# evanwang1990/FMwR

Hardware: AMD Instinct MI355X
Metric: training examples/sec, 10Mx1M sparse FM SGD (higher is better)
Workload: dtype f32

## Files before the change

fmwr_amd/_lib.py:

```python
import ctypes as C
import os

_PKG = os.path.dirname(os.path.abspath(__file__))
LIB_PATH = os.environ.get("FMX_LIB_PATH") or os.path.join(_PKG, "libfmx.so")

OK, ERR_INVALID, ERR_HIP, ERR_NOGPU, ERR_STATE = 0, 1, 2, 3, 4
TASK_CLASSIFICATION, TASK_REGRESSION, TASK_RANKING = 10, 20, 30
SOLVER_MCMC, SOLVER_ALS, SOLVER_SGD, SOLVER_FTRL, SOLVER_TDAP = 100, 200, 300, 500, 600
MODE_SEQUENTIAL, MODE_MINIBATCH = 0, 1
LINK_NONE, LINK_LOGISTIC, LINK_CLAMP, LINK_PROBIT = 0, 1, 2, 3
DIV_REL_SCORE, DIV_REL_MINMAX = 0, 1
SIM_COSINE, SIM_DOT = 0, 1
REDUCE_MEAN, REDUCE_SUM = 0, 1
COLUMNS_UNIFORM, COLUMNS_ZIPF = 1, 2
EVAL_LL, EVAL_AUC, EVAL_ACC, EVAL_RMSE, EVAL_MSE, EVAL_MAE = 0, 111, 222, 333, 444, 555
EVAL_PAIR_ACC, EVAL_BPR = 666, 777
KERNEL_ROWS_FORWARD, KERNEL_COLS_UPDATE, KERNEL_SCALAR, KERNEL_SEQ, KERNEL_ALS_SWEEP = 0, 1, 2, 3, 4

SYMBOLS = [
    "fmx_last_error", "fmx_device_count", "fmx_config_default", "fmx_engine_create", "fmx_engine_destroy", "fmx_set_params",
    "fmx_get_params", "fmx_engine_save", "fmx_engine_load", "fmx_matrix_from_rlist", "fmx_matrix_from_dgc", "fmx_matrix_from_csr", "fmx_matrix_synthetic", "fmx_matrix_synthetic_fields", "fmx_matrix_synthetic_iid", "fmx_matrix_synthetic_ragged", "fmx_matrix_synthetic_values", "fmx_train_stream", "fmx_matrix_set_labels", "fmx_matrix_set_fields", "fmx_matrix_destroy",
    "fmx_matrix_info", "fmx_matrix_export", "fmx_matrix_scales", "fmx_matrix_normalize", "fmx_predict", "fmx_train", "fmx_train_grid", "fmx_train_order", "fmx_num_batches",
    "fmx_step", "fmx_grad", "fmx_grad_buffer", "fmx_grad_elem_bytes", "fmx_grad_layout", "fmx_grad_begin", "fmx_grad_chunk", "fmx_apply_chunk", "fmx_apply", "fmx_sync", "fmx_stream", "fmx_predict_device",
    "fmx_als_plan_info", "fmx_als_tiled_info", "fmx_als_order_info", "fmx_als_carry_q", "fmx_als_vsweep", "fmx_mcmc_vsweep", "fmx_als_train", "fmx_mcmc_train", "fmx_mcmc_train_from", "fmx_mcmc_v_hyper", "fmx_evaluate", "fmx_train_tracked", "fmx_trace_size", "fmx_trace_get", "fmx_trace_params",
# ... 19 lines not shown
]
COLUMNS_BY_ROWS, COLUMNS_BY_ENTRIES = 0, 1
RARE_DROP, RARE_BUCKET = 0, 1
COMBINE_KEEP, COMBINE_SUM, COMBINE_FIRST = 0, 1, 2
COLUMN_DROP = 0xFFFFFFFF
SPLIT_ROWS, SPLIT_WITHIN_GROUPS, SPLIT_GROUPS = 0, 1, 2
SPLIT_ORDER_HASH, SPLIT_ORDER_TAIL = 0, 1
SPLIT_NO_PART = 0xFFFFFFFF
MET_VALUES, MET_COUNTS = 6, 4
MET_AUC, MET_LOGLOSS, MET_ACCURACY, MET_BRIER, MET_MEAN_PRED, MET_MEAN_LABEL = 0, 1, 2, 3, 4, 5
MET_MSE, MET_RMSE, MET_MAE, MET_MEAN_ERR = 0, 1, 2, 3
MET_ROWS, MET_POSITIVES, MET_PAIRS2, MET_CORRECT = 0, 1, 2, 3
CAL_NONE, CAL_PLATT, CAL_STEPS = 0, 1, 2
BINS_WIDTH, BINS_MASS = 0, 1
CAL_VALUES = 4
CAL_ECE, CAL_MCE, CAL_BRIER, CAL_LOGLOSS = 0, 1, 2, 3


TEST_HOOKS = ["fmx_debug_fail_next_plan_build", "fmx_debug_fail_next_comm_init", "fmx_debug_lose_next_seq_multiplier", "fmx_debug_stall_next_persistent_sweep",
              "fmx_debug_contrib_summary_chunk", "fmx_debug_foldin_slab", "fmx_debug_heldout_limits", "fmx_debug_pairs_hard_chunk", "fmx_debug_lists_limits", "fmx_debug_diversify_limits", "fmx_debug_neighbors_limits", "fmx_debug_interactions_limits", "fmx_debug_metrics_limits", "fmx_debug_take_limits", "fmx_debug_calibrate_limits", "fmx_debug_columns_limits", "fmx_debug_matrix_flags", "fmx_debug_cols_launches",
              "fmx_debug_long_launches", "fmx_debug_rows_launches", "fmx_debug_rows_merged_launches",
              "fmx_debug_rows_sched_launches", "fmx_debug_rows_sched_id_limit", "fmx_debug_rows_sched_export",
              "fmx_debug_rows_pace_launches", "fmx_debug_rows_pace_trace",
              "fmx_debug_rows_clock_launches", "fmx_debug_rows_clock_records_of", "fmx_debug_rows_clock_poison"]


class Config(C.Structure):
    _fields_ = [
        ("struct_size", C.c_uint32), ("task", C.c_int32), ("solver", C.c_int32), ("num_factor", C.c_int32),
        ("keep_w0", C.c_int32), ("keep_w1", C.c_int32),
        ("l2_w0", C.c_double), ("l1_w1", C.c_double), ("l2_w1", C.c_double), ("l1_v", C.c_double), ("l2_v", C.c_double),
        ("learn_rate", C.c_double),
        ("alpha_w", C.c_double), ("alpha_v", C.c_double), ("beta_w", C.c_double), ("beta_v", C.c_double),
        ("random_step", C.c_int32), ("mode", C.c_int32), ("batch_rows", C.c_int64),
        ("min_target", C.c_double), ("max_target", C.c_double),
        ("device", C.c_int32), ("batch_reduce", C.c_int32), ("gamma", C.c_double), ("tile_rows", C.c_int64),
        ("state_fp64", C.c_int32), ("exchange_chunks", C.c_int32), ("n_gpus", C.c_int32), ("als_max_levels", C.c_int32), ("seq_reassociate", C.c_int32), ("gpus_share_device", C.c_int32),
    ]


class FieldsSpec(C.Structure):
    _fields_ = [("struct_size", C.c_uint32), ("n_dense", C.c_int32), ("n_fields", C.c_int32), ("reserved", C.c_int32),
                ("field_vocab", C.c_void_p), ("skew", C.c_double), ("seed", C.c_uint64)]


class TrackConfig(C.Structure):
    _fields_ = [("struct_size", C.c_uint32), ("metric", C.c_int32), ("step_size", C.c_int64), ("convergence", C.c_double),
# ... 103 lines not shown
```

fmwr_amd/csrc/fm_batch_kernels.hip:

```cpp
#include <atomic>
#include <mutex>
#include <utility>
#include <vector>

#include "fmx_internal.h"
#include "fm_probit.h"
#include "fmx_test_hooks.h"

#ifndef FMX_U
#define FMX_U 4
#endif
#ifndef FMX_SPARSE_WAVES
#define FMX_SPARSE_WAVES 4
#endif
#ifndef FMX_DENSE_WAVES
#define FMX_DENSE_WAVES 4
#endif
#ifndef FMX_U_LARGE
#define FMX_U_LARGE 4
#endif
#ifndef FMX_U_SMALL
#define FMX_U_SMALL 8
#endif

// ... 2134 lines not shown
    }
  } else {
    const uint32_t* pr = a.brow + t_first;
    const float* pv = a.bval + t_first;
    while (rem > 0) {
      uint32_t r[FMX_U], x[FMX_U];
      ids(pr, pv, rem, r, x);
      round(rem, r, x);
      pr += FMX_U; pv += FMX_U;
      rem = rem > FMX_U ? rem - FMX_U : 0u;
    }
  }
  slice_get(v_raw, vf);
  ST* gtail = exchange_tail<ST, LPR>(T);
  double rows = a.global_rows;
  if (a.apply && a.load_gbuf && rows <= 0.0) rows = tail_get_rows(gtail);

  if (have) cols_finish<ST, LPR, KIND, false>(a, h, T, j, lig, vf, s, rows, I0 + gid, &w_pre);

  if (blockIdx.x == 0 && a.scalar != SCALAR_NONE)
    scalar_update(T.partials, T.n_partials, T.scal, T.scal_out, gtail, h, a.global_rows, a.scalar, red_g, red_q);
}

constexpr int LONG_STRIDE(int kp) { return 2 * kp + 4; }

template <typename ST, int LPR, bool NEED_Q>
__global__ __launch_bounds__(WG_THREADS) void fm_cols_long_partial_k(LongArgs la, ColsArgs a, ColsTables<ST> T) {
  using vec_t = typename Slice<ST>::vec;
  constexpr int VEC = Slice<ST>::N;
  constexpr int KP = LPR * VEC;
  constexpr int NSUB = 64 / LPR;
  const int lane = threadIdx.x & 63;
  const int64_t seg = (int64_t)blockIdx.x * (WG_THREADS / 64) + (threadIdx.x >> 6);
  if (seg >= la.n_seg) return;
  const int sub = lane / LPR, lig = lane % LPR;
  const int64_t j = la.lfeat[la.seg_feat[seg]];
  if (j < (int64_t)a.f0 || j >= (int64_t)a.f1) return;
  const int64_t ta = la.seg_begin[seg], tb = la.seg_end[seg];
  double vf[VEC];
  slice_get(*reinterpret_cast<const vec_t*>(T.V + ((size_t)j << RowStride<ST, LPR>::v(T.vsh)) + lig * VEC), vf);
  CoordSums s;
  sums_zero(s);
  const ST* __restrict__ St = T.S + lig * VEC;
  for (int64_t t = ta + sub; t < tb; t += (int64_t)NSUB * FMX_U) {
    uint32_t r[FMX_U], xb[FMX_U];
    float x[FMX_U];
// ... 144 lines not shown
  dim3 g1((unsigned)((la.n_seg + (WG_THREADS / 64) - 1) / (WG_THREADS / 64))), g2((unsigned)((la.n_long + (WG_THREADS / 64) - 1) / (WG_THREADS / 64)));
  const bool sparse_form = a.direct && !a.load_gbuf && !a.store_gbuf;
  static const bool side_ok = [] { const char* v = getenv("FMX_LONG_SIDE"); return !(v && v[0] == '0'); }();
  const bool side = lng && sparse_form && side_ok && la.n_seg >= 2048;
  hipStream_t ls = e->stream;
  if (side) {
    if (!e->side) {
      FMX_HIP(hipStreamCreateWithFlags(&e->side, hipStreamNonBlocking));
      FMX_HIP(hipEventCreateWithFlags(&e->side_fork, hipEventDisableTiming));
      FMX_HIP(hipEventCreateWithFlags(&e->side_join, hipEventDisableTiming));
    }
    FMX_HIP(hipEventRecord(e->side_fork, e->stream));
    FMX_HIP(hipStreamWaitEvent(e->side, e->side_fork, 0));
    ls = e->side;
  }
#define FMX_COLS_CASE(L)                                                                                        \
  case L:                                                                                                       \
    if (side) {                                                                                                 \
      g_long_launches[1]++;                                                                                     \
      hipLaunchKernelGGL((fm_cols_long_partial_k<ST, L, NQ>), g1, b, 0, ls, la, a, T);                          \
      hipLaunchKernelGGL((fm_cols_long_finish_k<ST, L, KIND>), g2, b, 0, ls, la, a, e->hyper, T);               \
    }                                                                                                           \
    if (sparse_form) {                                                                                          \
      if (!launch_lean<ST, L, KIND>(lists, g, b, e->stream, a, e->hyper, T)) {                                  \
        g_cols_launches[0]++;                                                                                   \
        hipLaunchKernelGGL((fm_cols_update_k<ST, L, KIND, true>), g, b, 0, e->stream, a, e->hyper, T);          \
      }                                                                                                         \
    }                                                                                                           \
    else hipLaunchKernelGGL((fm_cols_update_k<ST, L, KIND>), g, b, 0, e->stream, a, e->hyper, T);                \
    if (lng && !side) {                                                                                         \
      g_long_launches[0]++;                                                                                     \
      hipLaunchKernelGGL((fm_cols_long_partial_k<ST, L, NQ>), g1, b, 0, e->stream, la, a, T);                   \
      hipLaunchKernelGGL((fm_cols_long_finish_k<ST, L, KIND>), g2, b, 0, e->stream, la, a, e->hyper, T);        \
    }                                                                                                           \
    break;
  switch (lpr) {
    FMX_COLS_CASE(1) FMX_COLS_CASE(2) FMX_COLS_CASE(4) FMX_COLS_CASE(8)
    FMX_COLS_CASE(16) FMX_COLS_CASE(32) FMX_COLS_CASE(64)
    default: FMX_CHECK(false, FMX_ERR_INVALID, "unsupported padded factor count %d", mb_kp(e));
  }
#undef FMX_COLS_CASE
  if (side) {
    FMX_HIP(hipEventRecord(e->side_join, e->side));
    FMX_HIP(hipStreamWaitEvent(e->stream, e->side_join, 0));
  }
  FMX_HIP(hipGetLastError());
  return FMX_OK;
// ... 227 lines not shown
```

fmwr_amd/csrc/fm_ingest.hip:

```cpp
#include <hip/hip_runtime.h>

#include <atomic>
#include <mutex>
#include <thread>
#include <type_traits>
#include <vector>
#include <cstring>

#include <rocprim/rocprim.hpp>

#include "fmx_internal.h"

namespace fmx {

static std::atomic<int> g_fail_next_plan_build{0};
void debug_fail_next_plan_build() { g_fail_next_plan_build.store(1); }

__device__ __forceinline__ uint32_t entry_row(const int64_t* __restrict__ row_ptr, int64_t r0, int64_t nrows, int64_t base, int64_t t, int fixed_len) {
  if (fixed_len > 0) return (uint32_t)((t - base) / fixed_len);
  int64_t lo = r0, hi = r0 + nrows;
  while (hi - lo > 1) {
    const int64_t mid = (lo + hi) >> 1;
    if (row_ptr[mid] <= t) lo = mid; else hi = mid;
  }
// ... 982 lines not shown
  if (mb_wide(e)) {
    const int64_t total = n * (kp / 2 + 1);
    const dim3 g((unsigned)((total + 255) / 256)), b(256);
    if (unpack) hipLaunchKernelGGL((rows_pack_k<double, 2, true>), g, b, 0, e->stream, e->dV, e->dw, kp, kp, 1, d_ids, n, (double*)d_rows);
    else hipLaunchKernelGGL((rows_pack_k<double, 2, false>), g, b, 0, e->stream, e->dV, e->dw, kp, kp, 1, d_ids, n, (double*)d_rows);
  } else {
    const int64_t total = n * (kp / 4 + 1);
    const dim3 g((unsigned)((total + 255) / 256)), b(256);
    float* wb = (float*)mb_wbase(e);
    if (unpack) hipLaunchKernelGGL((rows_pack_k<float, 4, true>), g, b, 0, e->stream, e->V, wb, kp, mb_vstride(e), mb_wstride(e), d_ids, n, (float*)d_rows);
    else hipLaunchKernelGGL((rows_pack_k<float, 4, false>), g, b, 0, e->stream, e->V, wb, kp, mb_vstride(e), mb_wstride(e), d_ids, n, (float*)d_rows);
  }
  FMX_HIP(hipGetLastError());
  return FMX_OK;
}

void drop_plans(fmx_matrix* m) {
  for (auto& t : m->plans) plan_free(t);
  m->plans.clear();
  m->step_first_tile.clear();
  (void)hipFree(m->brow); (void)hipFree(m->bval);
  m->brow = nullptr; m->bval = nullptr;
  rows_sched_free(m);
  m->batch_rows = 0; m->tile_rows = 0; m->n_batches = 0; m->max_long_seg = 0; m->max_tile_cnt = 0;
  m->plan_generation++;
}

__global__ void gather_rows_k(const int64_t* __restrict__ src, const int64_t* __restrict__ rows, int64_t count, int64_t* __restrict__ dst) {
  const int64_t i = (int64_t)blockIdx.x * blockDim.x + threadIdx.x;
  if (i < count) dst[i] = src[rows[i]];
}

int build_batch_csc(fmx_matrix* m, int64_t batch_rows, int64_t tile_rows, hipStream_t stream) {
  FMX_CHECK(batch_rows > 0 && tile_rows > 0, FMX_ERR_INVALID, "batch_rows and tile_rows must be positive");
  if (m->batch_rows == batch_rows && m->tile_rows == tile_rows && !m->plans.empty()) return FMX_OK;
  FMX_HIP(hipSetDevice(m->device));
  drop_plans(m);
  const int64_t nb = (m->n + batch_rows - 1) / batch_rows;
  std::vector<int64_t> tile_start, step_first((size_t)nb + 1, 0);
  for (int64_t s = 0; s < nb; ++s) {
    step_first[(size_t)s] = (int64_t)tile_start.size();
    const int64_t end = (s + 1) * batch_rows < m->n ? (s + 1) * batch_rows : m->n;
    for (int64_t r = s * batch_rows; r < end; r += tile_rows) tile_start.push_back(r);
  }
  step_first[(size_t)nb] = (int64_t)tile_start.size();
  tile_start.push_back(m->n);
// ... 285 lines not shown
                            (uint32_t*)nullptr, (const uint32_t*)(d_dir + S.tile_dir[t]), S.words + S.tile_words[t]);
  }
  FMX_HIP(hipGetLastError());
  FMX_HIP(hipStreamSynchronize(stream));
  clock_gettime(CLOCK_MONOTONIC, &t1);
  S.build_ms = 1e3 * (double)(t1.tv_sec - t0.tv_sec) + 1e-6 * (double)(t1.tv_nsec - t0.tv_nsec);
  rows_sched_count_build();
  return FMX_OK;
}

int debug_rows_sched_export(const fmx_matrix* m, int64_t tile, int64_t block, uint32_t* out, int64_t cap_words, int64_t* steps) {
  const auto& S = m->rows_sched;
  FMX_CHECK(steps != nullptr, FMX_ERR_INVALID, "steps is NULL");
  *steps = -1;
  if (!S.words || S.generation != m->plan_generation || tile < 0 || tile >= (int64_t)S.tile_words.size() || S.tile_words[(size_t)tile] < 0) return FMX_OK;
  const int64_t blocks = (m->plans[(size_t)tile].nrows + 255) / 256;
  FMX_CHECK(block >= 0 && block < blocks, FMX_ERR_INVALID, "block %lld out of range (0..%lld)", (long long)block, (long long)blocks - 1);
  FMX_HIP(hipSetDevice(m->device));
  uint32_t d[2];
  FMX_HIP(hipMemcpy(d, S.dir + S.tile_dir[(size_t)tile] + block, sizeof(d), hipMemcpyDeviceToHost));
  const int64_t n = (int64_t)d[1] - (int64_t)d[0];
  *steps = n / 64 - (S.policy == SCHED_DEAL ? 1 : 0);
  FMX_CHECK(out != nullptr && n <= cap_words, FMX_ERR_INVALID, "the block's %lld words do not fit %lld", (long long)n, (long long)cap_words);
  if (n > 0) FMX_HIP(hipMemcpy(out, S.words + S.tile_words[(size_t)tile] + d[0], (size_t)n * sizeof(uint32_t), hipMemcpyDeviceToHost));
  return FMX_OK;
}

struct MergeWs {
  int64_t cap = 0;
  int n_parts_cap = 0;
  uint32_t *keys_in = nullptr, *keys_out = nullptr, *pos_in = nullptr, *pos_out = nullptr, *roff = nullptr, *rfeat = nullptr, *dcount = nullptr;
  uint32_t* blk = nullptr;
  void* sort_temp = nullptr; size_t sort_bytes = 0;
};

void merge_ws_free(MergeWs* w) {
  if (!w) return;
  (void)hipFree(w->keys_in); (void)hipFree(w->keys_out); (void)hipFree(w->pos_in); (void)hipFree(w->pos_out); (void)hipFree(w->roff);
  (void)hipFree(w->rfeat); (void)hipFree(w->dcount); (void)hipFree(w->blk); (void)hipFree(w->sort_temp);
  delete w;
}

static int merge_ws_reserve(fmx_engine* e, int64_t total, int n_parts) {
  if (!e->merge) e->merge = new MergeWs();
  MergeWs& w = *e->merge;
  if (total <= w.cap && n_parts <= w.n_parts_cap) return FMX_OK;
// ... 1002 lines not shown
```

fmwr_amd/csrc/fmx_api.hip:

```cpp
#include <algorithm>
#include <cmath>
#include <cstdlib>
#include <cstring>
#include <ctime>
#include <atomic>
#include <memory>

#include "fmx_internal.h"
#include "fmx_test_hooks.h"
#include "fm_probit.h"

namespace fmx {

static thread_local std::string g_error;

void set_error(const char* fmt, ...) {
  char buf[1024];
  va_list ap;
  va_start(ap, fmt);
  vsnprintf(buf, sizeof(buf), fmt, ap);
  va_end(ap);
  g_error = buf;
}

// ... 339 lines not shown
}

static int cols_args(fmx_engine* e, fmx_matrix* m, const TileRun& t, bool sparse_ok, ColsArgs* out) {
  const auto& pl = m->plans[(size_t)t.tile];
  ColsArgs c{};
  c.brow = m->brow + pl.base;
  c.bval = m->bval + pl.base;
  c.rows_active = (uint32_t)t.nrows;
  c.walk = 1;
  c.unit = m->unit_values;
  if (pl.feat && sparse_ok) {
    c.tfeat = pl.feat; c.toff = pl.soff; c.n_tfeat = pl.n_lists;
    c.trow0 = pl.row0; c.tval0 = pl.val0;
    c.list_entries = pl.cnt;
  } else {
    if (!pl.off) FMX_TRY(plan_ensure_dense(m, t.tile, e->stream));
    c.bptr = m->plans[(size_t)t.tile].off;
    c.list_entries = m->plans[(size_t)t.tile].cnt;
  }
  *out = c;
  return FMX_OK;
}

static int long_args(fmx_engine* e, fmx_matrix* m, int64_t tile, LongArgs* la, ColsArgs* c) {
  const auto& pl = m->plans[(size_t)tile];
  if (pl.n_long == 0) return FMX_OK;
  const int64_t need = m->max_long_seg * (2 * (int64_t)mb_kp(e) + 4);
  if (need > e->long_partial_cap) {
    FMX_HIP(hipStreamSynchronize(e->stream));
    (void)hipFree(e->long_partial); e->long_partial = nullptr; e->long_partial_cap = 0;
    FMX_HIP(hipMalloc(&e->long_partial, (size_t)need * sizeof(double)));
    e->long_partial_cap = need;
  }
  *la = LongArgs{pl.lfeat, pl.lpos, pl.lseg_ptr, pl.seg_list, pl.seg_begin, pl.seg_end, e->long_partial, (int64_t)pl.n_long, (int64_t)pl.n_seg};
  c->long_min = list_long_min();
  return FMX_OK;
}

static int run_step(fmx_engine* e, fmx_matrix* m, int64_t batch, int64_t rows_limit, bool finish_local, bool empty_share = false) {
  std::vector<TileRun> tiles;
  int64_t step_rows = 0;
  FMX_TRY(step_tiles(e, m, batch, rows_limit, &tiles, &step_rows));
  if (empty_share) { tiles.clear(); step_rows = 0; }
  if (tiles.empty()) {
    if (finish_local) return FMX_OK;
    tiles.push_back({m->step_first_tile[(size_t)batch], 0, 0});
  }
  const bool single = tiles.size() == 1;
  if (!(single && finish_local)) FMX_TRY(ensure_gbuf(e));
  int64_t partials = 0;
  for (size_t i = 0; i < tiles.size(); ++i) {
    int64_t np = 0;
    FMX_TRY(rows_phase(e, m, tiles[i], step_rows, partials, &np));
    partials += np;
    const bool last = i + 1 == tiles.size();
    ColsArgs c{};
    FMX_TRY(cols_args(e, m, tiles[i], single && finish_local, &c));
    c.load_gbuf = i > 0;
    c.store_gbuf = !(last && finish_local);
    c.apply = last && finish_local;
    c.scalar = !last ? SCALAR_NONE : (finish_local ? SCALAR_FUSED : SCALAR_PUBLISH);
    c.n_partials = last ? partials : 0;
    c.global_rows = (double)step_rows;
    LongArgs la{};
    FMX_TRY(long_args(e, m, tiles[i].tile, &la, &c));
    FMX_TRY(launch_cols_update(e, c, la));
  }
  return FMX_OK;
}

static int grad_begin(fmx_engine* e, fmx_matrix* m, int64_t batch, int64_t rows_limit) {
  std::vector<TileRun> tiles;
  int64_t step_rows = 0;
  FMX_TRY(step_tiles(e, m, batch, rows_limit, &tiles, &step_rows));
  FMX_TRY(ensure_gbuf(e));
  const int64_t cap = e->cfg.batch_rows < m->n ? e->cfg.batch_rows : (m->n > 0 ? m->n : 1);
  FMX_TRY(ensure_workspace(e, cap, cap, (int64_t)tiles.size()));
  e->open_tiles.clear();
  int64_t partials = 0, s_row0 = 0;
  for (const TileRun& t : tiles) {
// ... 1567 lines not shown
  debug_take_limits(fixed_entries, group_entries, rows_per_launch);
  return FMX_OK;
}
int fmx_debug_long_launches(int64_t* out) {
  FMX_CHECK(out != nullptr, FMX_ERR_INVALID, "out is NULL");
  debug_long_launches(out);
  return FMX_OK;
}
int fmx_debug_rows_launches(int64_t* out) {
  FMX_CHECK(out != nullptr, FMX_ERR_INVALID, "out is NULL");
  debug_rows_launches(out);
  return FMX_OK;
}
int fmx_debug_rows_merged_launches(int64_t* out) {
  FMX_CHECK(out != nullptr, FMX_ERR_INVALID, "out is NULL");
  debug_rows_merged_launches(out);
  return FMX_OK;
}
int fmx_debug_rows_sched_launches(int64_t* out) {
  FMX_CHECK(out != nullptr, FMX_ERR_INVALID, "out is NULL");
  debug_rows_sched_launches(out);
  return FMX_OK;
}
int fmx_debug_rows_pace_launches(int64_t* out) {
  FMX_CHECK(out != nullptr, FMX_ERR_INVALID, "out is NULL");
  debug_rows_pace_launches(out);
  return FMX_OK;
}
int fmx_debug_rows_clock_launches(int64_t* out) {
  FMX_CHECK(out != nullptr, FMX_ERR_INVALID, "out is NULL");
  debug_rows_clock_launches(out);
  return FMX_OK;
}
int fmx_debug_rows_clock_records_of(fmx_engine* e, int32_t replica, uint64_t* out) {
  FMX_CHECK(e != nullptr && out != nullptr, FMX_ERR_INVALID, "NULL engine or out");
  fmx_engine* r = group_replica(e, replica);
  FMX_CHECK(r != nullptr, FMX_ERR_INVALID, "no replica %d", (int)replica);
  FMX_HIP(hipSetDevice(r->cfg.device));
  const int st = debug_rows_clock_records(r, out);
  (void)hipSetDevice(e->cfg.device);
  return st;
}
int fmx_debug_rows_clock_poison(fmx_engine* e, uint32_t value) {
  FMX_CHECK(e != nullptr && value != 0u, FMX_ERR_INVALID, "NULL engine, or a target of 0 (which means none)");
  for (int i = 0; group_replica(e, i) != nullptr; ++i) { fmx_engine* r = group_replica(e, i); r->rows_clock_poisoned = 1; r->rows_clock_poison = value; }
  return FMX_OK;
// ... 62 lines not shown
```

fmwr_amd/csrc/fmx_internal.h:

```cpp
#pragma once
#include <hip/hip_runtime.h>

#include <cstdarg>
#include <cstdint>
#include <cstdio>
#include <cstdlib>
#include <functional>
#include <string>
#include <utility>
#include <vector>

#include "../../include/fmx.h"

namespace fmx {

void set_error(const char* fmt, ...);

#define FMX_HIP(call)                                                                         \
  do {                                                                                        \
    hipError_t _e = (call);                                                                   \
    if (_e != hipSuccess) {                                                                   \
      fmx::set_error("%s failed: %s (%s:%d)", #call, hipGetErrorString(_e), __FILE__, __LINE__); \
      return FMX_ERR_HIP;                                                                     \
    }                                                                                         \
// ... 110 lines not shown
    uint32_t* own_counts = nullptr;
    int64_t own_counts_h[17] = {0};
    void* own_pool = nullptr;
    uint32_t own_cap = 0;
  };
  std::vector<TilePlan> plans;
  uint64_t value_generation = 0;
  uint64_t plan_generation = 0;
  int64_t max_long_seg = 0;
  int64_t max_tile_cnt = 0;
  uint32_t* brow = nullptr;
  float* bval = nullptr;
  struct RowsSched {
    uint32_t* words = nullptr;
    uint32_t* dir = nullptr;
    std::vector<int64_t> tile_words;
    std::vector<int64_t> tile_dir;
    int policy = -1;
    uint64_t generation = 0;
    int tried = 0;
    size_t bytes = 0;
    double build_ms = 0.0;
  } rows_sched;
  int refilled_in_place = 0;
  int64_t* col_ptr = nullptr;
  uint32_t* crow = nullptr;
  float* cval = nullptr;
  uint32_t* als_feats = nullptr;
  std::vector<int64_t> als_level_ptr;
  uint32_t* als_heavy = nullptr;
  std::vector<int64_t> als_heavy_ptr;
  uint32_t* als_vh = nullptr;
  uint32_t* als_vh_seg0 = nullptr;
  uint32_t* als_vseg_feat = nullptr;
  int64_t* als_vseg_b = nullptr;
  int64_t* als_vseg_e = nullptr;
  double* als_vh_work = nullptr;
  int64_t als_n_vh = 0, als_n_vseg = 0;
  std::vector<int64_t> als_vh_ptr, als_vseg_ptr;
  std::vector<int32_t> als_level_of;
  int als_approx = 0;
  int als_coloured = 0;
  std::vector<int64_t> als_level_maxlen;
  int als_force_exact = 0;
  int als_plan_cap = -1;
  int64_t* als_level_ptr_dev = nullptr;
// ... 208 lines not shown
  if (lists == 0 || pl.n_long == 0) return 1;
  return ((uint64_t)pl.cnt <= 32ull * lists && (uint64_t)pl.n_long * 1024ull >= lists) ? 2 : 1;
}
int launch_rows_forward(fmx_engine* e, const RowsArgs& a, bool train, bool fp64_tables);
enum RowsSchedPolicy : int { SCHED_MERGE = 0, SCHED_DEAL = 3 };
constexpr int SCHED_STAGE_STEPS = 144;
constexpr uint32_t SCHED_BUBBLE = 0xFFFFFFFFu;
constexpr uint32_t SCHED_MAX_P = (1u << 30) - 1;
bool rows_sched_wanted(fmx_engine* e, const RowsArgs& a, int* policy);
void rows_sched_count_build();
void debug_rows_sched_launches(int64_t out[3]);
constexpr int PACE_TRACE_WORDS = 16;
constexpr int CLK_LINE = 16;
constexpr int CLK_WORDS = 3 * 8 * CLK_LINE;
constexpr int CLK_TICK_BITS = 40;
void debug_rows_pace_launches(int64_t out[2]);
void debug_rows_clock_launches(int64_t out[2]);
int debug_rows_clock_records(fmx_engine* e, uint64_t out[48]);
int debug_rows_pace_trace(fmx_engine* e, uint64_t* out, int64_t cap_words, int64_t* waves);
int rows_sched_build(fmx_matrix* m, int policy, hipStream_t stream);
void rows_sched_free(fmx_matrix* m);
void debug_rows_sched_id_limit(uint32_t limit);
int debug_rows_sched_export(const fmx_matrix* m, int64_t tile, int64_t block, uint32_t* out, int64_t cap_words, int64_t* steps);
int ensure_probit(fmx_engine* e);
int topk_run(fmx_engine* e, const fmx_matrix* C, int64_t r0, int64_t r1, const fmx_matrix* I, const fmx_matrix* X, int K, int link, int64_t* d_index,
             double* d_score);
int heldout_run(fmx_engine* e, const fmx_matrix* C, int64_t r0, int64_t r1, const fmx_matrix* I, const fmx_matrix* H, const fmx_matrix* X, int64_t* d_rank,
                double* d_score, const int32_t* ks, int n_ks, double* pc);
int heldout_means(fmx_engine* e, const double* pc, int64_t n, int cols, double* out, int64_t* counted);
void debug_heldout_limits(int window, int64_t chunk);
int lists_run(fmx_engine* e, const fmx_matrix* C, int64_t r0, int64_t r1, const fmx_matrix* I, const fmx_matrix* Lm, int link, int K, double* d_score,
              int64_t* d_pos, int64_t* d_index, double* d_tscore);
int project_run(fmx_engine* e, const fmx_matrix* m, int64_t r0, int64_t r1, bool with_w0, double* d_base, double* d_s);
void debug_lists_limits(int lds_entries, int64_t chunk);
int diversify_run(fmx_engine* e, const fmx_matrix* I, int64_t n, int P, const int64_t* index, const double* score, int K, double lambda, int relevance,
                  int64_t* oi, double* os, double* om, bool host);
void debug_diversify_limits(int lds_rows, int64_t chunk);
int neighbors_run(fmx_engine* e, const fmx_matrix* Q, int64_t r0, int64_t r1, const fmx_matrix* I, int K, int metric, bool skip_self, int64_t* d_index,
                  double* d_score);
void debug_neighbors_limits(int64_t slice_items, int64_t chunk_rows);
int contrib_run(fmx_engine* e, const fmx_matrix* m, int64_t r0, int64_t r1, double* d_out);
int pairs_build(const fmx_matrix* C, const fmx_matrix* I, const fmx_matrix* X, int n_neg, uint64_t seed, int64_t epoch, fmx_matrix** out,
                fmx_engine* e = nullptr, int n_cand = 1);
void debug_pairs_hard_chunk(int64_t contexts);
int contrib_summary_run(fmx_engine* e, const fmx_matrix* m, double* sum, double* abs_sum, int64_t* count);
int foldin_run(fmx_engine* e, const fmx_matrix* m, const uint32_t* ids, int64_t n_ids, double lw, double lv, int n_newton, bool pairs,
// ... 44 lines not shown
  const uint32_t* tfeat;
  const uint32_t* toff;
  uint32_t n_tfeat;
  const uint32_t* trow0;
  const uint32_t* tval0;
  int inline0;
  int walk;
  int load_gbuf;
  int store_gbuf;
  int apply;
  int scalar;
  int64_t n_partials;
  double global_rows;
  uint32_t f0, f1;
  int64_t s_row0;
  int store_compact;
  const uint32_t* rec_pos;
  int compact_tail;
  int unit;
  int direct;
  int64_t list_entries;
  int embed;
  int buf_gather;
};
struct LongArgs {
  const uint32_t* lfeat;
  const uint32_t* lpos;
  const uint32_t* lseg_ptr;
  const uint32_t* seg_feat;
  const uint32_t* seg_begin;
  const uint32_t* seg_end;
  double* partial;
  int64_t n_long, n_seg;
};
inline uint32_t list_long_min() {
  static const uint32_t v = [] { const char* s = getenv("FMX_LONG_MIN"); const long x = s ? atol(s) : 0; return x > 0 ? (uint32_t)x : 64u; }();
  return v;
}
constexpr int WIR_MAX_KP = 16;
constexpr uint32_t LIST_SEG = 1024;
int launch_cols_update(fmx_engine* e, const ColsArgs& a, const LongArgs& la);
constexpr int REC_PARTS_MAX = 64;
struct RecParts { int n; int64_t prefix[REC_PARTS_MAX + 1]; int64_t start[REC_PARTS_MAX]; };
int launch_record_keys(fmx_engine* e, const void* recs, const RecParts& parts, int64_t total, uint32_t* keys, uint32_t* pos);
int launch_apply_records(fmx_engine* e, const void* recs, const uint32_t* pos, const uint32_t* roff, const uint32_t* rfeat, const uint32_t* d_n,
                         int64_t max_lists, int64_t global_rows);
// ... 159 lines not shown
```

fmwr_amd/csrc/fmx_test_hooks.h:

```cpp
#ifndef FMX_TEST_HOOKS_H_
#define FMX_TEST_HOOKS_H_
#include <stdint.h>
#ifdef __cplusplus
extern "C" {
#endif
int fmx_debug_fail_next_plan_build(void);
int fmx_debug_fail_next_comm_init(void);
int fmx_debug_lose_next_seq_multiplier(void);
int fmx_debug_stall_next_persistent_sweep(void);
int fmx_debug_contrib_summary_chunk(int64_t entries);
int fmx_debug_foldin_slab(int64_t rows, int64_t groups);
int fmx_debug_heldout_limits(int32_t window, int64_t chunk);
int fmx_debug_pairs_hard_chunk(int64_t contexts);
int fmx_debug_lists_limits(int32_t lds_entries, int64_t chunk);
int fmx_debug_diversify_limits(int32_t lds_rows, int64_t chunk);
int fmx_debug_neighbors_limits(int64_t slice_items, int64_t chunk_rows);
int fmx_debug_interactions_limits(int32_t wave_entries, int32_t tile_entries, int64_t summary_rows_per_group);
int fmx_debug_metrics_limits(int32_t wave_rows, int32_t lds_rows, int64_t chunk_rows);
int fmx_debug_take_limits(int32_t fixed_entries, int32_t group_entries, int64_t rows_per_launch);
int fmx_debug_calibrate_limits(int64_t chunk_rows);
int fmx_debug_columns_limits(int32_t group_entries, int64_t chunk_entries, int64_t rows_per_launch);
int fmx_debug_matrix_flags(const fmx_matrix* m, int32_t* out );
int fmx_debug_cols_launches(int64_t* out);
int fmx_debug_long_launches(int64_t* out);
int fmx_debug_rows_launches(int64_t* out );
int fmx_debug_rows_merged_launches(int64_t* out );
int fmx_debug_rows_sched_launches(int64_t* out );
int fmx_debug_rows_sched_id_limit(uint32_t limit);
int fmx_debug_rows_sched_export(const fmx_matrix* m, int64_t tile, int64_t block, uint32_t* out, int64_t cap_words, int64_t* steps, int64_t* info );
int fmx_debug_rows_pace_launches(int64_t* out );
int fmx_debug_rows_clock_launches(int64_t* out );
int fmx_debug_rows_clock_records_of(fmx_engine* e, int32_t replica, uint64_t* out );
int fmx_debug_rows_clock_poison(fmx_engine* e, uint32_t value);
int fmx_debug_rows_pace_trace(fmx_engine* e, uint64_t* out, int64_t cap_words, int64_t* waves);
#ifdef __cplusplus
}
#endif
#endif
```

Baseline: 1.106 billion.

## Add precomputed column-stream schedule kernel for unit-valued k=16 SGD column updates

Adds a one-time per-plan build of an interleaved word stream that assigns each feature's row list to one of several slots per thread pair. The stream is ordered by row with a ramp so that loads of the row-side state are spread across time steps. A new column-update kernel reads that stream with unrolled prefetch and buffer loads, keeps V rows in LDS and per-slot gradient accumulators in registers, then calls the existing finish path. It targets the irregular gather and per-feature imbalance of the generic column kernel, in exchange for extra device memory, a build pass with host sync, and bubble padding in the stream.

New measurement: 1.116 billion (median of 6 runs). No clear change (+0.8%).

```diff
diff --git a/fmwr_amd/_lib.py b/fmwr_amd/_lib.py
--- a/fmwr_amd/_lib.py
+++ b/fmwr_amd/_lib.py
@@ -65,7 +65,8 @@
               "fmx_debug_long_launches", "fmx_debug_rows_launches", "fmx_debug_rows_merged_launches",
               "fmx_debug_rows_sched_launches", "fmx_debug_rows_sched_id_limit", "fmx_debug_rows_sched_export",
               "fmx_debug_rows_pace_launches", "fmx_debug_rows_pace_trace",
-              "fmx_debug_rows_clock_launches", "fmx_debug_rows_clock_records_of", "fmx_debug_rows_clock_poison"]
+              "fmx_debug_rows_clock_launches", "fmx_debug_rows_clock_records_of", "fmx_debug_rows_clock_poison",
+              "fmx_debug_cols_stream_launches", "fmx_debug_cols_stream_export"]
 
 
 class Config(C.Structure):
diff --git a/fmwr_amd/csrc/fm_batch_kernels.hip b/fmwr_amd/csrc/fm_batch_kernels.hip
--- a/fmwr_amd/csrc/fm_batch_kernels.hip
+++ b/fmwr_amd/csrc/fm_batch_kernels.hip
@@ -2180,6 +2180,156 @@
     scalar_update(T.partials, T.n_partials, T.scal, T.scal_out, gtail, h, a.global_rows, a.scalar, red_g, red_q);
 }
 
+#ifndef FMX_STREAM_WAVES
+#define FMX_STREAM_WAVES 3
+#endif
+template <int KIND, int U>
+__global__ __launch_bounds__(WG_THREADS, FMX_STREAM_WAVES) void fm_cols_stream_k(ColsArgs a, Hyper h, ColsTables<float> T) {
+  static_assert(KIND == UPD_SGD_L2 || KIND == UPD_SGD_L1, "the kinds without Q sums");
+  static_assert(WG_THREADS == 2 * STREAM_NG, "two lanes per stream");
+  constexpr int FB = STREAM_NG * STREAM_M;
+  __shared__ double red_g[WG_THREADS], red_q[WG_THREADS];
+  __shared__ float4 vrow[FB * 4];
+
+  const int tid = threadIdx.x;
+  const int g = tid >> 1, hl = tid & 1;
+  const int64_t p = (int64_t)a.f1;
+  const int64_t f0 = (int64_t)blockIdx.x * FB;
+#pragma unroll
+  for (int i = 0; i < FB * 4 / WG_THREADS; ++i) {
+    const int q = tid + i * WG_THREADS;
+    const int64_t f = f0 + (q >> 2) < p ? f0 + (q >> 2) : p - 1;
+    vrow[q] = *reinterpret_cast<const float4*>(T.V + ((size_t)f << RowStride<float, 4>::v(T.vsh)) + (q & 3) * 4);
+  }
+  __syncthreads();
+
+  double G[STREAM_M][8], Gw[STREAM_M];
+  int cnt[STREAM_M];
+#pragma unroll
+  for (int s = 0; s < STREAM_M; ++s) {
+    Gw[s] = 0.0; cnt[s] = 0;
+#pragma unroll
+    for (int i = 0; i < 8; ++i) G[s][i] = 0.0;
+  }
+  const uint32_t d0 = a.stream_dir[blockIdx.x], d1 = a.stream_dir[blockIdx.x + 1];
+  const uint32_t Tb = (d1 - d0) / (uint32_t)STREAM_NG;
+  const __amdgpu_buffer_rsrc_t s_rsrc = table_rsrc(T.S, (uint32_t)(T.s_rows * (16 * sizeof(float))));
+  auto words = [&](uint32_t t, uint32_t (&w)[U]) {
+#pragma unroll
+    for (int u = 0; u < U; ++u) {
+      const bool in = t + u < Tb;
+      const uint32_t v = a.stream_words[in ? d0 + (t + u) * (uint32_t)STREAM_NG + (uint32_t)g : 0u];
+      w[u] = in ? v : STREAM_BUBBLE;
+    }
+  };
+  uint32_t wn[U];
+  words(0, wn);
+  for (uint32_t t = 0; t < Tb; t += U) {
+    uint32_t w[U];
+#pragma unroll
+    for (int u = 0; u < U; ++u) w[u] = wn[u];
+    words(t + U, wn);
+    __builtin_amdgcn_sched_barrier(0);
+    float4 sa[U], sb[U];
+#pragma unroll
+    for (int u = 0; u < U; ++u) {
+      const bool live = w[u] != STREAM_BUBBLE;
+      const uint32_t off = (w[u] & ((1u << STREAM_SLOT_SHIFT) - 1u)) * 64u + (uint32_t)(hl * 16);
+      sa[u] = buf_row(s_rsrc, live ? off : BUF_SKIP, float());
+      sb[u] = buf_row(s_rsrc, live ? off + 32u : BUF_SKIP, float());
+    }
+#pragma unroll
+    for (int u = 0; u < U; ++u) {
+      const bool live = w[u] != STREAM_BUBBLE;
+      const int slot = (int)((w[u] >> STREAM_SLOT_SHIFT) & (uint32_t)(STREAM_M - 1));
+      auto strip = [](float4& v, int p0) {
+        const uint32_t ux = __float_as_uint(v.x), uy = __float_as_uint(v.y), uz = __float_as_uint(v.z), uw = __float_as_uint(v.w);
+        v.x = __uint_as_float(ux & ~3u); v.y = __uint_as_float(uy & ~3u); v.z = __uint_as_float(uz & ~3u); v.w = __uint_as_float(uw & ~3u);
+        return ((ux & 3u) << p0) | ((uy & 3u) << (p0 + 2)) | ((uz & 3u) << (p0 + 4)) | ((uw & 3u) << (p0 + 6));
+      };
+      const uint32_t part = strip(sa[u], 8 * hl) | strip(sb[u], 8 * hl + 16);
+      const float amul = __uint_as_float(group_or_dpp<2>(part));
+      const float4 va = vrow[((slot * STREAM_NG + g) << 2) + hl], vb = vrow[((slot * STREAM_NG + g) << 2) + hl + 2];
+      const double x = 1.0;
+      const double ax = (double)amul * x;
+      double sf[8], vf[8], gg[8];
+      slice_get(sa[u], sf); slice_get(sb[u], sf + 4);
+      slice_get(va, vf); slice_get(vb, vf + 4);
+#pragma unroll
+      for (int i = 0; i < 8; ++i) gg[i] = ax * (sf[i] - vf[i] * x);
+#pragma unroll
+      for (int s = 0; s < STREAM_M; ++s)
+        if (live && slot == s) {
+          Gw[s] += ax;
+          cnt[s] += 1;
+#pragma unroll
+          for (int i = 0; i < 8; ++i) G[s][i] += gg[i];
+        }
+    }
+  }
+  float* gtail = exchange_tail<float, 4>(T);
+  const double rows = a.global_rows;
+#pragma unroll
+  for (int s = 0; s < STREAM_M; ++s) {
+    const int64_t j = f0 + s * STREAM_NG + g;
+    if (j < p) {
+#pragma unroll
+      for (int c = 0; c < 2; ++c) {
+        const int lig = hl + 2 * c;
+        CoordSums cs;
+        sums_zero(cs);
+#pragma unroll
+        for (int i = 0; i < 4; ++i) cs.G[i] = G[s][4 * c + i];
+        cs.Gw = Gw[s];
+        cs.cnt = (double)cnt[s];
+        double vf[4];
+        slice_get(vrow[((s * STREAM_NG + g) << 2) + lig], vf);
+        cols_finish<float, 4, KIND, false>(a, h, T, j, lig, vf, cs, rows, j, nullptr);
+      }
+    }
+  }
+  if (blockIdx.x == 0 && a.scalar != SCALAR_NONE)
+    scalar_update(T.partials, T.n_partials, T.scal, T.scal_out, gtail, h, a.global_rows, a.scalar, red_g, red_q);
+}
+
+static std::atomic<int64_t> g_cols_stream[3];
+void debug_cols_stream_launches(int64_t out[3]) {
+  for (int i = 0; i < 3; ++i) out[i] = g_cols_stream[i].load();
+}
+void cols_stream_count_build() { g_cols_stream[2]++; }
+static int cols_stream_mode() {
+  static const int v = [] { const char* s = getenv("FMX_COLS_STREAM"); return s ? atoi(s) : 1; }();
+  return v;
+}
+constexpr int64_t STREAM_MIN_TABLE = 4 << 20;
+bool cols_stream_wanted(fmx_engine* e, const fmx_matrix* m, int64_t rows, int* rho_q) {
+  const int mode = cols_stream_mode();
+  if (mode == 0 || mb_wide(e) || e->kp32 != 16 || e->k != 16 || !m->unit_values || m->refilled_in_place) return false;
+  if (e->hyper.kind != UPD_SGD_L2 && e->hyper.kind != UPD_SGD_L1) return false;
+  if (e->cfg.task == FMX_TASK_RANKING || rows <= 0) return false;
+  if (mode != 2 && rows * (int64_t)(16 * sizeof(float)) <= STREAM_MIN_TABLE) return false;
+  static const int rho = [] { const char* s = getenv("FMX_COLS_STREAM_RHO"); const int v = s ? atoi(s) : 6; return v < 1 ? 1 : (v > 8 ? 8 : v); }();
+  *rho_q = rho;
+  return true;
+}
+template <typename ST, int L, int KIND>
+static bool launch_stream(fmx_engine* e, const LongArgs& la, dim3 b, hipStream_t st, const ColsArgs& a, const Hyper& h, const ColsTables<ST>& T) {
+  if constexpr (sizeof(ST) != 4 || L != 4 || !(KIND == UPD_SGD_L2 || KIND == UPD_SGD_L1)) {
+    return false;
+  } else {
+    if (a.stream_state == 0 || cols_stream_mode() == 0) return false;
+    if (!a.buf_gather || a.embed != EMBED_BITS || !a.unit || !a.direct || !a.apply || a.load_gbuf || a.store_gbuf || a.store_compact || a.f0 != 0 || a.f1 != e->p) return false;
+    if (a.stream_state != 1 || !a.stream_words || !a.stream_dir || a.tfeat || la.n_long != 0) { g_cols_stream[1]++; return false; }
+    static const int u2 = [] { const char* s = getenv("FMX_COLS_STREAM_U"); return s ? atoi(s) : 4; }();
+    dim3 g((unsigned)(((int64_t)e->p + STREAM_NG * STREAM_M - 1) / (STREAM_NG * STREAM_M)));
+    g_cols_stream[0]++;
+    if (u2 == 4) hipLaunchKernelGGL((fm_cols_stream_k<KIND, 4>), g, b, 0, st, a, h, T);
+    else if (u2 == 2) hipLaunchKernelGGL((fm_cols_stream_k<KIND, 2>), g, b, 0, st, a, h, T);
+    else hipLaunchKernelGGL((fm_cols_stream_k<KIND, 1>), g, b, 0, st, a, h, T);
+    return true;
+  }
+}
+
 constexpr int LONG_STRIDE(int kp) { return 2 * kp + 4; }
 
 template <typename ST, int LPR, bool NEED_Q>
@@ -2370,7 +2520,8 @@
       hipLaunchKernelGGL((fm_cols_long_finish_k<ST, L, KIND>), g2, b, 0, ls, la, a, e->hyper, T);               \
     }                                                                                                           \
     if (sparse_form) {                                                                                          \
-      if (!launch_lean<ST, L, KIND>(lists, g, b, e->stream, a, e->hyper, T)) {                                  \
+      if (launch_stream<ST, L, KIND>(e, la, b, e->stream, a, e->hyper, T)) {                                    \
+      } else if (!launch_lean<ST, L, KIND>(lists, g, b, e->stream, a, e->hyper, T)) {                           \
         g_cols_launches[0]++;                                                                                   \
         hipLaunchKernelGGL((fm_cols_update_k<ST, L, KIND, true>), g, b, 0, e->stream, a, e->hyper, T);          \
       }                                                                                                         \
diff --git a/fmwr_amd/csrc/fm_ingest.hip b/fmwr_amd/csrc/fm_ingest.hip
--- a/fmwr_amd/csrc/fm_ingest.hip
+++ b/fmwr_amd/csrc/fm_ingest.hip
@@ -1028,6 +1028,7 @@
   (void)hipFree(m->brow); (void)hipFree(m->bval);
   m->brow = nullptr; m->bval = nullptr;
   rows_sched_free(m);
+  cols_stream_free(m);
   m->batch_rows = 0; m->tile_rows = 0; m->n_batches = 0; m->max_long_seg = 0; m->max_tile_cnt = 0;
   m->plan_generation++;
 }
@@ -1359,6 +1360,166 @@
   const int64_t n = (int64_t)d[1] - (int64_t)d[0];
   *steps = n / 64 - (S.policy == SCHED_DEAL ? 1 : 0);
   FMX_CHECK(out != nullptr && n <= cap_words, FMX_ERR_INVALID, "the block's %lld words do not fit %lld", (long long)n, (long long)cap_words);
+  if (n > 0) FMX_HIP(hipMemcpy(out, S.words + S.tile_words[(size_t)tile] + d[0], (size_t)n * sizeof(uint32_t), hipMemcpyDeviceToHost));
+  return FMX_OK;
+}
+
+template <bool WRITE>
+__global__ __launch_bounds__(STREAM_NG) void cols_stream_k(const uint32_t* __restrict__ off, const uint32_t* __restrict__ brow, uint32_t p, uint32_t nrows, uint32_t tr,
+                                                           uint32_t* __restrict__ steps, const uint32_t* __restrict__ dir, uint32_t* __restrict__ words) {
+  const uint32_t g = threadIdx.x, b = blockIdx.x;
+  uint32_t pos[STREAM_M], end[STREAM_M];
+  bool bad = false;
+#pragma unroll
+  for (int u = 0; u < STREAM_M; ++u) {
+    const uint64_t f = (uint64_t)b * (STREAM_NG * STREAM_M) + (uint64_t)u * STREAM_NG + g;
+    pos[u] = 0; end[u] = 0;
+    if (f < p) { pos[u] = off[f]; end[u] = off[f + 1]; }
+    bad = bad || end[u] - pos[u] > (uint32_t)STREAM_MAX_LIST;
+  }
+  if (bad) {
+#pragma unroll
+    for (int u = 0; u < STREAM_M; ++u) end[u] = pos[u];
+  }
+  uint32_t T = 0, next = 0;
+  uint32_t* out = nullptr;
+  if constexpr (WRITE) {
+    T = (dir[b + 1] - dir[b]) / STREAM_NG;
+    out = words + dir[b] + g;
+  }
+  int64_t t = -1;
+  for (;;) {
+    int sel = -1;
+    uint32_t best = 0;
+#pragma unroll
+    for (int u = 0; u < STREAM_M; ++u)
+      if (pos[u] < end[u]) {
+        const uint32_t r = brow[pos[u]];
+        if (sel < 0 || r < best) { sel = u; best = r; }
+      }
+    if (sel < 0) break;
+#pragma unroll
+    for (int u = 0; u < STREAM_M; ++u)
+      if (u == sel) pos[u] += 1;
+    const int64_t fs = ((int64_t)best * tr + nrows - 1) / nrows - 1;
+    t = t + 1 > fs ? t + 1 : fs;
+    if constexpr (WRITE) {
+      if (t < (int64_t)T) {
+        for (; next < (uint32_t)t; ++next) out[(size_t)next * STREAM_NG] = STREAM_BUBBLE;
+        out[(size_t)t * STREAM_NG] = best | ((uint32_t)sel << STREAM_SLOT_SHIFT);
+        next = (uint32_t)t + 1;
+      }
+    }
+  }
+  if constexpr (WRITE) {
+    for (; next < T; ++next) out[(size_t)next * STREAM_NG] = STREAM_BUBBLE;
+  } else {
+    atomicMax(&steps[b], (bad || t + 1 > (int64_t)STREAM_STEP_CAP) ? (uint32_t)STREAM_STEP_CAP + 1 : (uint32_t)(t + 1));
+  }
+}
+
+void cols_stream_free(fmx_matrix* m) {
+  (void)hipFree(m->cols_stream.words);
+  (void)hipFree(m->cols_stream.dir);
+  m->cols_stream = fmx_matrix::ColsStream{};
+}
+
+static inline int64_t stream_blocks(uint32_t p) { return ((int64_t)p + STREAM_NG * STREAM_M - 1) / (STREAM_NG * STREAM_M); }
+
+int cols_stream_build(fmx_matrix* m, int rho_q, hipStream_t stream) {
+  auto& S = m->cols_stream;
+  if (S.tried && S.generation == m->plan_generation && S.rho_q == rho_q) return FMX_OK;
+  cols_stream_free(m);
+  S.tried = 1; S.generation = m->plan_generation; S.rho_q = rho_q;
+  const size_t nt = m->plans.size();
+  S.tile_words.assign(nt, -1);
+  S.tile_dir.assign(nt, 0);
+  FMX_CHECK(rho_q >= 1 && rho_q <= 8, FMX_ERR_INVALID, "cols_stream_build: utilisation %d/8", rho_q);
+  if (m->refilled_in_place || nt == 0 || !m->unit_values || m->p == 0) return FMX_OK;
+  const int64_t blocks = stream_blocks(m->p);
+  auto eligible = [&](const fmx_matrix::TilePlan& pl) {
+    return pl.off && pl.off_in_pool && !pl.feat && pl.n_long == 0 && pl.nrows > 0 && pl.nrows <= (1LL << STREAM_SLOT_SHIFT) && pl.cnt > 0 && pl.cnt < (1LL << 32);
+  };
+  auto ramp = [&](const fmx_matrix::TilePlan& pl) {
+    const int64_t d = blocks * STREAM_NG * rho_q;
+    const int64_t tr = (8 * pl.cnt + d - 1) / d;
+    return (uint32_t)(tr > 1 ? tr : 1);
+  };
+  bool any = false;
+  int64_t slots = 0;
+  for (size_t t = 0; t < nt; ++t) { S.tile_dir[t] = slots; slots += blocks + 1; any = any || eligible(m->plans[t]); }
+  if (!any) return FMX_OK;
+  FMX_HIP(hipSetDevice(m->device));
+  timespec t0, t1;
+  clock_gettime(CLOCK_MONOTONIC, &t0);
+  uint32_t* d_dir = nullptr;
+  FMX_HIP(hipMalloc(&d_dir, (size_t)slots * sizeof(uint32_t)));
+  S.dir = d_dir;
+  FMX_HIP(hipMemsetAsync(d_dir, 0, (size_t)slots * sizeof(uint32_t), stream));
+  for (size_t t = 0; t < nt; ++t) {
+    const auto& pl = m->plans[t];
+    if (!eligible(pl)) continue;
+    hipLaunchKernelGGL((cols_stream_k<false>), dim3((unsigned)blocks), dim3(STREAM_NG), 0, stream, (const uint32_t*)pl.off, (const uint32_t*)(m->brow + pl.base), m->p,
+                       (uint32_t)pl.nrows, ramp(pl), d_dir + S.tile_dir[t] + 1, (const uint32_t*)nullptr, (uint32_t*)nullptr);
+  }
+  FMX_HIP(hipGetLastError());
+  std::vector<uint32_t> h((size_t)slots);
+  FMX_HIP(hipMemcpyAsync(h.data(), d_dir, (size_t)slots * sizeof(uint32_t), hipMemcpyDeviceToHost, stream));
+  FMX_HIP(hipStreamSynchronize(stream));
+  int64_t total = 0;
+  any = false;
+  for (size_t t = 0; t < nt; ++t) {
+    if (!eligible(m->plans[t])) continue;
+    uint32_t* d = h.data() + S.tile_dir[t];
+    bool fits = true;
+    int64_t words = 0;
+    for (int64_t b = 1; b <= blocks; ++b) { fits = fits && d[b] <= (uint32_t)STREAM_STEP_CAP; words += (int64_t)d[b] * STREAM_NG; }
+    if (!fits || words >= (1LL << 31)) continue;
+    uint32_t at = 0;
+    for (int64_t b = 1; b <= blocks; ++b) { const uint32_t steps = d[b]; d[b - 1] = at; at += steps * (uint32_t)STREAM_NG; }
+    d[blocks] = at;
+    S.tile_words[t] = total;
+    total += at;
+    any = true;
+  }
+  if (!any) return FMX_OK;
+  FMX_HIP(hipMemcpyAsync(d_dir, h.data(), (size_t)slots * sizeof(uint32_t), hipMemcpyHostToDevice, stream));
+  if (hipMalloc(&S.words, (size_t)(total > 0 ? total : 1) * sizeof(uint32_t)) != hipSuccess) {
+    (void)hipGetLastError();
+    FMX_HIP(hipStreamSynchronize(stream));
+    (void)hipFree(S.dir);
+    S.words = nullptr; S.dir = nullptr;
+    S.tile_words.assign(nt, -1);
+    return FMX_OK;
+  }
+  S.bytes = (size_t)(total > 0 ? total : 1) * sizeof(uint32_t) + (size_t)slots * sizeof(uint32_t);
+  for (size_t t = 0; t < nt; ++t) {
+    if (S.tile_words[t] < 0) continue;
+    const auto& pl = m->plans[t];
+    hipLaunchKernelGGL((cols_stream_k<true>), dim3((unsigned)blocks), dim3(STREAM_NG), 0, stream, (const uint32_t*)pl.off, (const uint32_t*)(m->brow + pl.base), m->p,
+                       (uint32_t)pl.nrows, ramp(pl), (uint32_t*)nullptr, (const uint32_t*)(d_dir + S.tile_dir[t]), S.words + S.tile_words[t]);
+  }
+  FMX_HIP(hipGetLastError());
+  FMX_HIP(hipStreamSynchronize(stream));
+  clock_gettime(CLOCK_MONOTONIC, &t1);
+  S.build_ms = 1e3 * (double)(t1.tv_sec - t0.tv_sec) + 1e-6 * (double)(t1.tv_nsec - t0.tv_nsec);
+  cols_stream_count_build();
+  return FMX_OK;
+}
+
+int debug_cols_stream_export(const fmx_matrix* m, int64_t tile, int64_t block, uint32_t* out, int64_t cap_words, int64_t* steps) {
+  const auto& S = m->cols_stream;
+  FMX_CHECK(steps != nullptr, FMX_ERR_INVALID, "steps is NULL");
+  *steps = -1;
+  if (!S.words || S.generation != m->plan_generation || tile < 0 || tile >= (int64_t)S.tile_words.size() || S.tile_words[(size_t)tile] < 0) return FMX_OK;
+  const int64_t blocks = stream_blocks(m->p);
+  FMX_CHECK(block >= 0 && block < blocks, FMX_ERR_INVALID, "block %lld out of range (0..%lld)", (long long)block, (long long)blocks - 1);
+  FMX_HIP(hipSetDevice(m->device));
+  uint32_t d[2];
+  FMX_HIP(hipMemcpy(d, S.dir + S.tile_dir[(size_t)tile] + block, sizeof(d), hipMemcpyDeviceToHost));
+  const int64_t n = (int64_t)d[1] - (int64_t)d[0];
+  *steps = n / STREAM_NG;
+  FMX_CHECK((out != nullptr || n == 0) && n <= cap_words, FMX_ERR_INVALID, "the block's %lld words do not fit %lld", (long long)n, (long long)cap_words);
   if (n > 0) FMX_HIP(hipMemcpy(out, S.words + S.tile_words[(size_t)tile] + d[0], (size_t)n * sizeof(uint32_t), hipMemcpyDeviceToHost));
   return FMX_OK;
 }
diff --git a/fmwr_amd/csrc/fmx_api.hip b/fmwr_amd/csrc/fmx_api.hip
--- a/fmwr_amd/csrc/fmx_api.hip
+++ b/fmwr_amd/csrc/fmx_api.hip
@@ -385,6 +385,22 @@
   return FMX_OK;
 }
 
+static int cols_stream_args(fmx_engine* e, fmx_matrix* m, const TileRun& t, ColsArgs* c) {
+  int rho_q = 0;
+  if (!cols_stream_wanted(e, m, t.nrows, &rho_q)) return FMX_OK;
+  FMX_TRY(cols_stream_build(m, rho_q, e->stream));
+  c->stream_state = 2;
+  const auto& S = m->cols_stream;
+  const auto& pl = m->plans[(size_t)t.tile];
+  if (S.words && S.dir && S.generation == m->plan_generation && (size_t)t.tile < S.tile_words.size() && S.tile_words[(size_t)t.tile] >= 0 && pl.r0 == t.r0 &&
+      pl.nrows == t.nrows && c->bptr && c->bptr == pl.off && pl.off_in_pool) {
+    c->stream_words = S.words + S.tile_words[(size_t)t.tile];
+    c->stream_dir = S.dir + S.tile_dir[(size_t)t.tile];
+    c->stream_state = 1;
+  }
+  return FMX_OK;
+}
+
 static int long_args(fmx_engine* e, fmx_matrix* m, int64_t tile, LongArgs* la, ColsArgs* c) {
   const auto& pl = m->plans[(size_t)tile];
   if (pl.n_long == 0) return FMX_OK;
@@ -419,6 +435,7 @@
     const bool last = i + 1 == tiles.size();
     ColsArgs c{};
     FMX_TRY(cols_args(e, m, tiles[i], single && finish_local, &c));
+    if (single && finish_local && tiles[i].nrows > 0) FMX_TRY(cols_stream_args(e, m, tiles[i], &c));
     c.load_gbuf = i > 0;
     c.store_gbuf = !(last && finish_local);
     c.apply = last && finish_local;
@@ -2032,6 +2049,16 @@
   debug_rows_sched_launches(out);
   return FMX_OK;
 }
+int fmx_debug_cols_stream_launches(int64_t* out) {
+  FMX_CHECK(out != nullptr, FMX_ERR_INVALID, "out is NULL");
+  debug_cols_stream_launches(out);
+  return FMX_OK;
+}
+int fmx_debug_cols_stream_export(const fmx_matrix* m, int64_t tile, int64_t block, uint32_t* out, int64_t cap_words, int64_t* steps, int64_t* info) {
+  FMX_CHECK(m != nullptr, FMX_ERR_INVALID, "matrix is NULL");
+  if (info) { info[0] = (int64_t)m->cols_stream.bytes; info[1] = (int64_t)(m->cols_stream.build_ms * 1e3); info[2] = m->cols_stream.rho_q; info[3] = 0; }
+  return debug_cols_stream_export(m, tile, block, out, cap_words, steps);
+}
 int fmx_debug_rows_pace_launches(int64_t* out) {
   FMX_CHECK(out != nullptr, FMX_ERR_INVALID, "out is NULL");
   debug_rows_pace_launches(out);
diff --git a/fmwr_amd/csrc/fmx_internal.h b/fmwr_amd/csrc/fmx_internal.h
--- a/fmwr_amd/csrc/fmx_internal.h
+++ b/fmwr_amd/csrc/fmx_internal.h
@@ -156,6 +156,17 @@
     size_t bytes = 0;
     double build_ms = 0.0;
   } rows_sched;
+  struct ColsStream {
+    uint32_t* words = nullptr;
+    uint32_t* dir = nullptr;
+    std::vector<int64_t> tile_words;
+    std::vector<int64_t> tile_dir;
+    int rho_q = 0;
+    uint64_t generation = 0;
+    int tried = 0;
+    size_t bytes = 0;
+    double build_ms = 0.0;
+  } cols_stream;
   int refilled_in_place = 0;
   int64_t* col_ptr = nullptr;
   uint32_t* crow = nullptr;
@@ -410,6 +421,14 @@
 void rows_sched_free(fmx_matrix* m);
 void debug_rows_sched_id_limit(uint32_t limit);
 int debug_rows_sched_export(const fmx_matrix* m, int64_t tile, int64_t block, uint32_t* out, int64_t cap_words, int64_t* steps);
+constexpr int STREAM_NG = 128, STREAM_M = 4, STREAM_MAX_LIST = 64, STREAM_STEP_CAP = 512, STREAM_SLOT_SHIFT = 28;
+constexpr uint32_t STREAM_BUBBLE = 0xFFFFFFFFu;
+bool cols_stream_wanted(fmx_engine* e, const fmx_matrix* m, int64_t rows, int* rho_q);
+int cols_stream_build(fmx_matrix* m, int rho_q, hipStream_t stream);
+void cols_stream_free(fmx_matrix* m);
+void cols_stream_count_build();
+void debug_cols_stream_launches(int64_t out[3]);
+int debug_cols_stream_export(const fmx_matrix* m, int64_t tile, int64_t block, uint32_t* out, int64_t cap_words, int64_t* steps);
 int ensure_probit(fmx_engine* e);
 int topk_run(fmx_engine* e, const fmx_matrix* C, int64_t r0, int64_t r1, const fmx_matrix* I, const fmx_matrix* X, int K, int link, int64_t* d_index,
              double* d_score);
@@ -500,6 +519,9 @@
   int64_t list_entries;
   int embed;
   int buf_gather;
+  int stream_state;
+  const uint32_t* stream_words;
+  const uint32_t* stream_dir;
 };
 struct LongArgs {
   const uint32_t* lfeat;
diff --git a/fmwr_amd/csrc/fmx_test_hooks.h b/fmwr_amd/csrc/fmx_test_hooks.h
--- a/fmwr_amd/csrc/fmx_test_hooks.h
+++ b/fmwr_amd/csrc/fmx_test_hooks.h
@@ -33,6 +33,8 @@
 int fmx_debug_rows_clock_records_of(fmx_engine* e, int32_t replica, uint64_t* out );
 int fmx_debug_rows_clock_poison(fmx_engine* e, uint32_t value);
 int fmx_debug_rows_pace_trace(fmx_engine* e, uint64_t* out, int64_t cap_words, int64_t* waves);
+int fmx_debug_cols_stream_launches(int64_t* out );
+int fmx_debug_cols_stream_export(const fmx_matrix* m, int64_t tile, int64_t block, uint32_t* out, int64_t cap_words, int64_t* steps, int64_t* info );
 #ifdef __cplusplus
 }
 #endif
```
